# frankenz/Deep-convolutional-neural-network-ResNet-26-and-Attention-network

Measured on AMD Instinct MI355X. Metric: tiles/sec fwd+bwd, 256x256x3 bags, ResNet-26+attn, higher is better.
Workload: dtype bf16; 1 GPU; 8 bags x 256 tiles @256x256x3 per GPU, ResNet-26 (20/40/60/80) + attention-MIL head, fwd+bwd full-bag path (BASELINE.json configs[1]); global_bags=8, tiles_per_bag=256, tile=256, parallelism=bag-parallel dp1, one RCCL all-reduce of the flat 2.56 MB gradient bucket

## Files before the change

### deep-convolutional-neural-network-resnet-26-and-attention-network_amd/csrc/conv_bwd_fused.hip

```cpp
#include "pf_common.cuh"
#include "reduce.cuh"
#include <cstdlib>

struct BwdFusedArgs {
    const __bf16* dz;
    const __bf16* w;
    const __bf16* x;
    const __bf16* addend;
    __bf16* dx;
    float* slab;
    ConvGeom g;
    int ntiles;
    int lds_w_off, lds_x_off, lds_dump_off, lds_a2_off;
    int lds_x2_off;
    int apply_mask;
    float slope;
    unsigned z_bytes, x_bytes;
    unsigned g_bytes;
    int gpx;
    int xpx;
    unsigned long long* stamp;
};

#ifdef MIL_STAMP
// ... 399 lines not shown
                slab[(size_t)(mt * 16 + gq * 4 + e) * SLAB_COLS + nt * 16 + r] = wacc[i][nt][e];
        if (i == bias_i && r == 0) {
#pragma unroll
            for (int e = 0; e < 4; ++e) {
                const int row = mt * 16 + gq * 4 + e;
                const int co = row - CTAP * CZ;
                if (co >= 0 && co < CZ) slab[(size_t)MT * 16 * SLAB_COLS + co] = bacc[e];
            }
        }
    }
}


template <bool ADD, bool MASK>
__global__ __launch_bounds__(512, 4) void conv_bwd_fused16_kernel(BwdFusedArgs a) {
    extern __shared__ __attribute__((aligned(16))) char smem[];
    MIL_POISON(smem);
    constexpr int CZ = 24, NTX = 2, KS = 3, NW = 8;
    constexpr int PIXB = 48, PIXX = 48, CX = 24, HW = 18, ROWB = HW * PIXB;
    constexpr int KSTEPS_STD = 7;
    constexpr int NTHR = 512, MTW = 2, KSTEPS = MIL_K20_STEPS, MT = 12, MW = 2;
    constexpr int NPX = 4;
    constexpr int HALO0 = 16;
    const ConvGeom& g = a.g;
    const int tid = threadIdx.x, lane = tid & 63;
    const int wave = __builtin_amdgcn_readfirstlane(tid >> 6);
    const int r = lane & 15, gq = lane >> 4;
    char* ldsW = smem + a.lds_w_off;
    {
        mil_stage_filter(ldsW, reinterpret_cast<const char*>(a.w) + KSTEPS_STD * NTX * 64 * 16, KSTEPS * NTX * 64 * 16, tid, NTHR);
        if (tid < 2) *reinterpret_cast<u32x2_t*>(smem + tid * a.lds_a2_off + HALO0 + (HW * HW - 1) * PIXB + 40) = u32x2_t{0u, 0u};
    }
    const __amdgpu_buffer_rsrc_t rs_z = mil_rsrc(a.dz, a.z_bytes);
    const __amdgpu_buffer_rsrc_t rs_x = mil_rsrc(a.x, a.x_bytes);
    const __amdgpu_buffer_rsrc_t rs_add = mil_rsrc(a.addend, a.addend ? a.g_bytes : 0);
    const __amdgpu_buffer_rsrc_t rs_dx = mil_rsrc(a.dx, a.g_bytes);
    const int H = g.H, W = g.W, GPX = a.gpx;

    int h_pos[NPX];
    const int h_j8 = (tid & 3) * 8;
    const int h_lds0 = (tid >> 2) * PIXB + h_j8;
#pragma unroll
    for (int i = 0; i < NPX; ++i) {
        const int px = i < 3 ? (tid >> 2) + 128 * i : tid;
        const int hy = px / HW, hx = px - hy * HW;
        h_pos[i] = px < HW * HW ? (hy << 10) | hx : (int)0x80000000u;
    }
    u32x2_t rx[NPX];
    auto fetch_halo = [&](const TileOrigin& o) {
        const int iy0 = o.oy0 - 1, ix0 = o.ox0 - 1;
        const int base = ((o.img0 * H + iy0) * W + ix0) * GPX;
#pragma unroll
        for (int i = 0; i < NPX; ++i) {
            int p = h_pos[i];
            asm volatile("" : "+v"(p));
            const int hy = (p >> 10) & 1023, hx = p & 1023;
            const bool ok = (p >= 0) & ((unsigned)(iy0 + hy) < (unsigned)H) & ((unsigned)(ix0 + hx) < (unsigned)W);
            const int rel = (hy * W + hx) * GPX + (i < 3 ? h_j8 : 32);
            rx[i] = __builtin_amdgcn_raw_buffer_load_b64(rs_z, ok ? (unsigned)(base + rel) : MIL_OOB, 0, 0);
        }
    };

    auto koff = [](int q) { return mil_k20_off(q, ROWB, PIXB); };
    const int bA = (wave * MTW * HW + r) * PIXB + 16 * gq;
    int zb[KSTEPS];
#pragma unroll
    for (int sl = 0; sl < KSTEPS; ++sl) {
        const int o0 = koff(4 * sl);
        const int d1 = koff(4 * sl + 1) - o0 - 16, d2 = koff(4 * sl + 2) - o0 - 32, d3 = koff(4 * sl + 3) - o0 - 48;
        zb[sl] = bA + (gq == 1 ? d1 : gq == 2 ? d2 : gq == 3 ? d3 : 0);
    }
    const int e_ty = wave * MTW + (gq & 1);
    const int c_off = (gq >> 1) * 16;
    const int x_lds = (e_ty * 16 + r) * PIXX + c_off;
    const bool last_ok = (gq >> 1) == 0;
    const int q4 = (lane & 15) >> 2, p4 = lane & 3;
    int zw[MW][2];
    {
        const int kl0 = 8 * gq + q4, kl1 = kl0 + 4;
        const int wpl0 = ((kl0 >> 4) * HW + (kl0 & 15)) * PIXB, wpl1 = ((kl1 >> 4) * HW + (kl1 & 15)) * PIXB;
#pragma unroll
        for (int i = 0; i < MW; ++i) {
            int P = 4 * (wave + NW * i) + p4;
            if (P >= KS * KS * 5) P = 0;
            const int tap = P / 5, c4 = P - tap * 5;
            const int wt = ((tap / KS) * HW + (tap % KS)) * PIXB + c4 * 8;
            zw[i][0] = wpl0 + wt; zw[i][1] = wpl1 + wt;
        }
    }
    const int xb = (8 * gq + q4) * PIXX + p4 * 8;
    f32x4_t wacc[MW][NTX];
#pragma unroll
    for (int i = 0; i < MW; ++i)
#pragma unroll
        for (int nt = 0; nt < NTX; ++nt) wacc[i][nt] = f32x4_t{0.f, 0.f, 0.f, 0.f};

    TileWalker cur, nxt;
    const int bid = mil_xcd_block_id();
    cur.init(g, bid, gridDim.x);
    nxt = cur; nxt.advance();
    if (bid < a.ntiles) fetch_halo(cur.origin(g));
    unsigned goff = MIL_OOB, goff_n = MIL_OOB;
    u32x4_t rxc0, radd0;
    u32x2_t rxc1, radd1;
    auto fetch_x = [&](const TileOrigin& o) {
        const int opix = (o.img0 * H + o.oy0 + e_ty) * W + o.ox0 + r;
        const bool ok = e_ty < H - o.oy0 && r < W - o.ox0;
        const unsigned xoff = ok ? (unsigned)(opix * (CX * 2) + c_off) : MIL_OOB;
        goff_n = ok ? (unsigned)(opix * GPX + c_off) : MIL_OOB;
        rxc0 = __builtin_amdgcn_raw_buffer_load_b128(rs_x, xoff, 0, 0);
        rxc1 = __builtin_amdgcn_raw_buffer_load_b64(rs_x, last_ok ? xoff + 32 : MIL_OOB, 0, 0);
    };
    auto fetch_add = [&]() {
        if constexpr (ADD) {
            radd0 = __builtin_amdgcn_raw_buffer_load_b128(rs_add, goff_n, 0, 0);
            radd1 = __builtin_amdgcn_raw_buffer_load_b64(rs_add, last_ok ? goff_n + 32 : MIL_OOB, 0, 0);
        }
    };
    if (bid < a.ntiles) { fetch_x(cur.origin(g)); fetch_add(); }

    const int buf_step = a.lds_a2_off, xbuf_step = a.lds_x2_off;
    int buf = 0, xbuf = 0;
    MIL_ST_DECL
    for (int tile = bid; tile < a.ntiles; tile += gridDim.x) {
        MIL_ST_BEGIN()
        char* ldsA_t = smem + buf + HALO0;
        char* ldsX_t = smem + a.lds_x_off + xbuf;
        buf = buf_step - buf;
        xbuf = xbuf_step - xbuf;
        {
            int p2 = h_pos[2], p3 = h_pos[3];
            asm volatile("" : "+v"(p2), "+v"(p3));
            *reinterpret_cast<u32x2_t*>(ldsA_t + h_lds0) = rx[0];
            *reinterpret_cast<u32x2_t*>(ldsA_t + h_lds0 + 128 * PIXB) = rx[1];
            *reinterpret_cast<u32x2_t*>(ldsA_t + (p2 >= 0 ? h_lds0 + 256 * PIXB : -16)) = rx[2];
            const int l3 = p3 >= 0 ? tid * PIXB + 32 : -16;
            *reinterpret_cast<u32x2_t*>(ldsA_t + l3) = rx[3];
            *reinterpret_cast<u32x2_t*>(ldsA_t + (p3 >= 0 ? l3 - 40 : -8)) = rx[3];
        }
        *reinterpret_cast<u32x4_t*>(ldsX_t + x_lds) = rxc0;
        *reinterpret_cast<u32x4_t*>(last_ok ? ldsX_t + x_lds + 32 : smem + a.lds_dump_off) = u32x4_t{rxc1[0], rxc1[1], 0u, 0x3f800000u};
        goff = goff_n;
        MIL_ST_MARK(0)
        __syncthreads();
        MIL_ST_MARK(1)
        const bool more = tile + (int)gridDim.x < a.ntiles;
        if (more) { const TileOrigin o_next = nxt.origin(g); fetch_halo(o_next); fetch_x(o_next); }
        cur = nxt; nxt.advance();
        u32x4_t mk0;
        u32x2_t mk1;
        if constexpr (MASK) {
            mk0 = *reinterpret_cast<const u32x4_t*>(ldsX_t + x_lds);
            mk1 = *reinterpret_cast<const u32x2_t*>(last_ok ? ldsX_t + x_lds + 32 : smem + a.lds_dump_off);
        }

        f32x4_t acc[MTW][NTX];
#pragma unroll
        for (int m = 0; m < MTW; ++m)
#pragma unroll
            for (int nt = 0; nt < NTX; ++nt) acc[m][nt] = f32x4_t{0.f, 0.f, 0.f, 0.f};
        {
            Frag8<BF16> wc[NTX], zc[MTW], wn[NTX], zn[MTW];
#pragma unroll
            for (int nt = 0; nt < NTX; ++nt) wc[nt] = lds_frag<BF16>(ldsW + (nt * 64 + lane) * 16);
#pragma unroll
            for (int m = 0; m < MTW; ++m) zc[m] = lds_frag<BF16>(ldsA_t + zb[0] + koff(0) + m * ROWB);
#pragma unroll
            for (int sl = 0; sl < KSTEPS; ++sl) {
                if (sl + 1 < KSTEPS) {
#pragma unroll
                    for (int nt = 0; nt < NTX; ++nt) wn[nt] = lds_frag<BF16>(ldsW + (((sl + 1) * NTX + nt) * 64 + lane) * 16);
#pragma unroll
                    for (int m = 0; m < MTW; ++m) zn[m] = lds_frag<BF16>(ldsA_t + zb[sl + 1] + koff(4 * (sl + 1)) + m * ROWB);
                }
                __builtin_amdgcn_sched_barrier(0);
#pragma unroll
                for (int m = 0; m < MTW; ++m)
#pragma unroll
                    for (int nt = 0; nt < NTX; ++nt) acc[m][nt] = mma8(wc[nt], zc[m], acc[m][nt]);
                __builtin_amdgcn_sched_barrier(0);
#pragma unroll
                for (int nt = 0; nt < NTX; ++nt) wc[nt] = wn[nt];
#pragma unroll
                for (int m = 0; m < MTW; ++m) zc[m] = zn[m];
            }
        }
        MIL_ST_MARK(2)

        {
            float v[8];
#pragma unroll
            for (int i = 0; i < 4; ++i) {
                float lo = acc[0][0][i], hi = acc[1][0][i];
                if (i == 0) mil_swap16<true>(lo, hi); else mil_swap16<false>(lo, hi);
                v[i] = lo;
                v[4 + i] = hi;
            }
            if constexpr (ADD) {
                const bf16x8_t t = __builtin_bit_cast(bf16x8_t, radd0);
#pragma unroll
                for (int i = 0; i < 8; ++i) v[i] += (float)t[i];
            }
            if constexpr (MASK) {
                const bf16x8_t t = __builtin_bit_cast(bf16x8_t, mk0);
#pragma unroll
                for (int i = 0; i < 8; ++i) v[i] *= ((float)t[i] > 0.f ? 1.f : a.slope);
            }
            bf16x8_t ov;
#pragma unroll
            for (int i = 0; i < 8; ++i) ov[i] = (__bf16)v[i];
            __builtin_amdgcn_raw_buffer_store_b128(__builtin_bit_cast(u32x4_t, ov), rs_dx, goff, 0, 0);
        }
        {
            float v[4];
#pragma unroll
            for (int i = 0; i < 4; ++i) {
                float lo = acc[0][1][i], hi = acc[1][1][i];
                if (i == 0) mil_swap16<true>(lo, hi); else mil_swap16<false>(lo, hi);
                v[i] = lo;
            }
            if constexpr (ADD) {
                const bf16x4_t t = __builtin_bit_cast(bf16x4_t, radd1);
#pragma unroll
                for (int i = 0; i < 4; ++i) v[i] += (float)t[i];
            }
            if constexpr (MASK) {
                const bf16x4_t t = __builtin_bit_cast(bf16x4_t, mk1);
#pragma unroll
                for (int i = 0; i < 4; ++i) v[i] *= ((float)t[i] > 0.f ? 1.f : a.slope);
            }
            bf16x4_t ov;
#pragma unroll
            for (int i = 0; i < 4; ++i) ov[i] = (__bf16)v[i];
            const u32x2_t ou = __builtin_bit_cast(u32x2_t, ov);
            const unsigned off = last_ok ? goff + 32 : MIL_OOB;
            if (GPX == 48) __builtin_amdgcn_raw_buffer_store_b128(u32x4_t{ou[0], ou[1], 0u, 0u}, rs_dx, off, 0, 0);
            else __builtin_amdgcn_raw_buffer_store_b64(ou, rs_dx, off, 0, 0);
        }
        MIL_ST_MARK(3)
        if (more) fetch_add();
        MIL_ST_MARK(4)

        {
            bf16x8_t xc[NTX], zc[MW], xn[NTX], zn[MW];
#pragma unroll
            for (int nt = 0; nt < NTX; ++nt) xc[nt] = mil_tr_pair(ldsX_t + xb + nt * 32, ldsX_t + xb + nt * 32 + 4 * PIXX);
#pragma unroll
            for (int i = 0; i < MW; ++i) zc[i] = mil_tr_pair(ldsA_t + zw[i][0], ldsA_t + zw[i][1]);
#pragma unroll
            for (int kk = 0; kk < 8; ++kk) {
                if (kk + 1 < 8) {
#pragma unroll
                    for (int nt = 0; nt < NTX; ++nt)
                        xn[nt] = mil_tr_pair(ldsX_t + xb + (kk + 1) * 32 * PIXX + nt * 32, ldsX_t + xb + (kk + 1) * 32 * PIXX + nt * 32 + 4 * PIXX);
#pragma unroll
                    for (int i = 0; i < MW; ++i)
                        zn[i] = mil_tr_pair(ldsA_t + zw[i][0] + (kk + 1) * 2 * ROWB, ldsA_t + zw[i][1] + (kk + 1) * 2 * ROWB);
                }
                __builtin_amdgcn_sched_barrier(0);
#pragma unroll
                for (int i = 0; i < MW; ++i) {
                    if (i == MW - 1 && wave + NW * i >= MT) continue;
#pragma unroll
                    for (int nt = 0; nt < NTX; ++nt)
                        wacc[i][nt] = __builtin_amdgcn_mfma_f32_16x16x32_bf16(zc[i], xc[nt], wacc[i][nt], 0, 0, 0);
                }
                __builtin_amdgcn_sched_barrier(0);
#pragma unroll
                for (int nt = 0; nt < NTX; ++nt) xc[nt] = xn[nt];
#pragma unroll
                for (int i = 0; i < MW; ++i) zc[i] = zn[i];
            }
        }
        MIL_ST_MARK(5)
#ifdef MIL_STAMP
        ++st_tiles;
#endif
    }
#ifdef MIL_STAMP
    if (a.stamp && lane == 0) {
        unsigned long long* d = a.stamp + ((size_t)blockIdx.x * NW + wave) * 8;
#pragma unroll
        for (int i = 0; i < 6; ++i) d[i] = st_sum[i];
        d[6] = (unsigned long long)st_tiles;
        d[7] = __builtin_amdgcn_s_memrealtime() - st_rt0;
    }
#endif
    constexpr int SLAB_COLS = NTX * 16;
    constexpr size_t SLAB_ELEMS = (size_t)(14 + 1) * 16 * SLAB_COLS;
    float* slab = a.slab + (size_t)blockIdx.x * SLAB_ELEMS;
#pragma unroll
    for (int i = 0; i < MW; ++i) {
        const int mt = wave + NW * i;
        if (mt >= MT) continue;
#pragma unroll
        for (int nt = 0; nt < NTX; ++nt)
#pragma unroll
            for (int e = 0; e < 4; ++e)
                slab[(size_t)(mt * 16 + gq * 4 + e) * SLAB_COLS + nt * 16 + r] = wacc[i][nt][e];
    }
}

#include "conv_bwd_fused16_x3.cuh"


template <typename T, int CZ, int NTX, int KS, int NW = 4>
static int run_bwd_fused(BwdFusedArgs a, float* dw, float* db, void* ws, size_t ws_bytes, int cout, int cin, int accumulate, bool query,
                         size_t* need, hipStream_t stream, bool dense_grads = false) {
    constexpr int ESZ = T::ESZ, EM = ESZ / 2;
    constexpr int PIXB = mil_pix_pitch(CZ, ESZ);
    constexpr int CX = mil_nt_to_cp(NTX);
    constexpr int PIXX = mil_pix_pitch(CX, ESZ);
    constexpr int DUMPA = T::SPLIT ? CZ * 2 + 16 : 16, DUMPX = T::SPLIT ? CX * 2 + 16 : 16;
    constexpr int KSTEPS = (KS * KS * (CZ / 8) + 3) / 4;
    constexpr int RG = KS * KS * (CZ / 8);
    constexpr int MT = (RG + 1) / 2;
    mil_geom_tiles(a.g, 8);
    {
        const int px = (a.g.hh * a.g.hw) << a.g.ti_log2;
        const int need = ((px * PIXB + 15) & ~15) + DUMPA + KSTEPS * NTX * 64 * 8 * ESZ + 256 * PIXX + DUMPX;
        if (need > 160 * 1024 && a.g.tw_log2 == 3 && a.g.ti_log2 == 2 && (a.g.Wo > 8 || a.g.Ho > 8)) mil_geom_set(a.g, 4, 4, 0);
    }
    const int halo_px = (a.g.hh * a.g.hw) << a.g.ti_log2;
    if (halo_px > 400 || a.g.hh >= 1024 || a.g.hw >= 1024) return MIL_ERR_UNSUPPORTED;
    const size_t img_bytes = (size_t)a.g.H * a.g.W * (CZ > CX ? CZ : CX) * ESZ;
    int chunk = mil_imgs_under_2g(img_bytes);
    if (chunk >= 16) chunk &= ~15;
    const int n_total = a.g.n_img;
    if (chunk < n_total) { a.g.n_img = chunk; a.g.n_groups = (chunk + (1 << a.g.ti_log2) - 1) >> a.g.ti_log2; }
    const int a_bytes = ((halo_px * PIXB + 15) & ~15) + DUMPA;
    const int w_bytes = KSTEPS * NTX * 64 * 8 * ESZ;
    const int x_bytes = 256 * PIXX;
    const bool dbuf = 2 * (2 * a_bytes + w_bytes + x_bytes + DUMPX) <= 160 * 1024;
    bool t16 = false;
    if constexpr (CZ == 24 && NTX == 2 && KS == 3 && NW == 8 && !T::SPLIT)
        t16 = dbuf && a.g.tw_log2 == 4 && a.g.th_log2 == 4 && a.g.ti_log2 == 0 && a.g.H < 1024 && a.g.W < 1024 &&
              cout == 20;
    if (dense_grads && !t16) return MIL_ERR_UNSUPPORTED;
    const int lds = (dbuf ? 2 : 1) * a_bytes + w_bytes + (t16 ? 2 : 1) * x_bytes + DUMPX;
    if (lds > 160 * 1024) return MIL_ERR_UNSUPPORTED;
    const int ntiles = a.g.n_groups * a.g.tiles_y * a.g.tiles_x;
    auto kern = a.addend ? (a.apply_mask ? conv_bwd_fused_kernel<T, CZ, NTX, KS, true, true, NW> : conv_bwd_fused_kernel<T, CZ, NTX, KS, true, false, NW>)
                         : (a.apply_mask ? conv_bwd_fused_kernel<T, CZ, NTX, KS, false, true, NW> : conv_bwd_fused_kernel<T, CZ, NTX, KS, false, false, NW>);
    if constexpr (CZ == 24 && NTX == 2 && KS == 3 && NW == 8 && !T::SPLIT) {
        if (t16) kern = a.addend ? (a.apply_mask ? conv_bwd_fused16_kernel<true, true> : conv_bwd_fused16_kernel<true, false>)
                                 : (a.apply_mask ? conv_bwd_fused16_kernel<false, true> : conv_bwd_fused16_kernel<false, false>);
    }
    if (lds > 64 * 1024) {
        if (hipFuncSetAttribute(reinterpret_cast<const void*>(kern), hipFuncAttributeMaxDynamicSharedMemorySize, lds) != hipSuccess)
            return MIL_ERR_LAUNCH;
    }
    int per_cu = 3;
    {
        int o1 = mil_resident_per_cu(conv_bwd_fused_kernel<T, CZ, NTX, KS, true, true, NW>, lds, 3, 64 * NW);
        int o2 = mil_resident_per_cu(conv_bwd_fused_kernel<T, CZ, NTX, KS, false, true, NW>, lds, 3, 64 * NW);
        int o3 = mil_resident_per_cu(conv_bwd_fused_kernel<T, CZ, NTX, KS, true, false, NW>, lds, 3, 64 * NW);
        if constexpr (CZ == 24 && NTX == 2 && KS == 3 && NW == 8 && !T::SPLIT) {
            if (t16) {
                o1 = mil_resident_per_cu(conv_bwd_fused16_kernel<true, true>, lds, 3, 512);
                o2 = mil_resident_per_cu(conv_bwd_fused16_kernel<false, true>, lds, 3, 512);
                o3 = mil_resident_per_cu(conv_bwd_fused16_kernel<true, false>, lds, 3, 512);
            }
        }
        per_cu = o1 < o2 ? o1 : o2; per_cu = per_cu < o3 ? per_cu : o3;
    }
    int grid = mil_num_cus() * per_cu;
    if (grid > ntiles) grid = ntiles;
    const size_t slab_elems = (size_t)(MT + 1) * 16 * NTX * 16;
    size_t bytes = slab_elems * grid * sizeof(float);
#ifdef MIL_STAMP
    const size_t stamp_off = (bytes + 15) & ~(size_t)15;
    bytes = stamp_off + (size_t)grid * NW * 8 * sizeof(unsigned long long);
#endif
    if (query) { *need = bytes; return MIL_OK; }
    if (!ws || ws_bytes < bytes) return MIL_ERR_ARG;
#ifdef MIL_STAMP
    a.stamp = reinterpret_cast<unsigned long long*>(reinterpret_cast<char*>(ws) + stamp_off);
#endif
    const int a_tot = (dbuf ? 2 : 1) * a_bytes;
    a.slab = (float*)ws; a.lds_w_off = a_tot; a.lds_x_off = a_tot + w_bytes; a.lds_dump_off = a_tot + w_bytes + x_bytes * (t16 ? 2 : 1);
    a.lds_a2_off = dbuf ? a_bytes : 0;
    a.lds_x2_off = t16 ? x_bytes : 0;
    if (grid <= 0) return MIL_OK;
    const int n_rows = KS * KS * CZ;
    const BwdFusedArgs a0 = a;
    for (int i0 = 0; i0 < n_total; i0 += chunk) {
        const int n = n_total - i0 < chunk ? n_total - i0 : chunk;
        BwdFusedArgs c = a0;
        c.g.n_img = n;
        c.g.n_groups = (n + (1 << c.g.ti_log2) - 1) >> c.g.ti_log2;
        c.ntiles = c.g.n_groups * c.g.tiles_y * c.g.tiles_x;
        const int gz = dense_grads ? 20 : CZ, gx = dense_grads ? 20 : CX;
        const size_t zo = (size_t)i0 * a.g.H * a.g.W * gz, xo = (size_t)i0 * a.g.H * a.g.W * CX, go = (size_t)i0 * a.g.H * a.g.W * gx;
        c.dz = a0.dz + zo * EM; c.x = a0.x + xo * EM; c.dx = a0.dx + go * EM;
        if (a0.addend) c.addend = a0.addend + go * EM;
        c.z_bytes = (unsigned)((size_t)n * a.g.H * a.g.W * gz * ESZ);
        c.x_bytes = (unsigned)((size_t)n * a.g.H * a.g.W * CX * ESZ);
        c.g_bytes = (unsigned)((size_t)n * a.g.H * a.g.W * gx * ESZ);
        c.gpx = gz * 2;
        int gr = grid < c.ntiles ? grid : c.ntiles;
        hipLaunchKernelGGL(kern, dim3(gr), dim3(64 * NW), lds, stream, c);
        MIL_CHECK_LAUNCH();
        {
            MilReduceJob j{};
            j.slab = (const float*)ws; j.nslab = gr; j.slab_elems = slab_elems; j.slab_cols = NTX * 16; j.n_rows = n_rows;
            j.dw = dw; j.db = db; j.cout = cout; j.cin = cin; j.ks = KS; j.kind = 1; j.cinp = CZ;
            j.bias_off = t16 ? (KS * KS / 2) * CZ * NTX * 16 + (CX - 1) : MT * 16 * NTX * 16; j.bias_stride = t16 ? NTX * 16 : 1;
            if (t16) {
                j.cinp = 20; j.n_rows = KS * KS * 20; j.bias_off = (KS * KS / 2) * 20 * NTX * 16 + (CX - 1);
            }
            j.accumulate = (i0 > 0) ? 1 : accumulate;
            mil_reduce_or_defer(j, stream, chunk >= n_total);
        }
        MIL_CHECK_LAUNCH();
    }
    return MIL_OK;
}

static int run_bwd_fused16_x3(BwdFusedArgs a, float* dw, float* db, void* ws, size_t ws_bytes, int cout, int cin, int accumulate, bool query,
                              size_t* need, hipStream_t stream, bool dense_grads) {
    constexpr int KS = 3, NTX = 2, MT_PITCH = 14;
    if (cout != 20 || cin != 20) return MIL_ERR_UNSUPPORTED;
    mil_geom_tiles(a.g, 8);
    if (a.g.tw_log2 != 4 || a.g.th_log2 != 4 || a.g.ti_log2 != 0 || a.g.H >= 1024 || a.g.W >= 1024) return MIL_ERR_UNSUPPORTED;
    constexpr int A_PLANE = 16 + 18 * 18 * 48, X_PLANE = 256 * 48, W_BYTES = MIL_K20_STEPS * NTX * 64 * 32;
    constexpr int lds = 2 * A_PLANE + W_BYTES + 2 * X_PLANE + 64;
    const int gpx = dense_grads ? 80 : 96, xpx = 96;
    const size_t img_bytes = (size_t)a.g.H * a.g.W * 96;
    int chunk = mil_imgs_under_2g(img_bytes);
    if (chunk >= 16) chunk &= ~15;
    const int n_total = a.g.n_img;
    if (chunk < n_total) { a.g.n_img = chunk; a.g.n_groups = chunk; }
    const int ntiles = a.g.n_groups * a.g.tiles_y * a.g.tiles_x;
    auto pick = [](bool add, bool mask) {
        return add ? (mask ? conv_bwd_fused16x3_kernel<true, true> : conv_bwd_fused16x3_kernel<true, false>)
                   : (mask ? conv_bwd_fused16x3_kernel<false, true> : conv_bwd_fused16x3_kernel<false, false>);
    };
    auto kern = pick(a.addend != nullptr, a.apply_mask != 0);
    static std::atomic<unsigned long long> attr_set{0};
    if (mil_device_needs(attr_set)) {
        for (int v = 0; v < 4; ++v)
            if (hipFuncSetAttribute(reinterpret_cast<const void*>(pick(v & 1, v & 2)), hipFuncAttributeMaxDynamicSharedMemorySize, lds) != hipSuccess)
                return MIL_ERR_LAUNCH;
        mil_device_done(attr_set);
    }
    int per_cu = 3;
    for (int v = 0; v < 4; ++v) {
        const int o = mil_resident_per_cu(pick(v & 1, v & 2), lds, 3, 256);
        per_cu = o < per_cu ? o : per_cu;
    }
    int grid = mil_num_cus() * per_cu;
    if (grid > ntiles) grid = ntiles;
    const size_t slab_elems = (size_t)(MT_PITCH + 1) * 16 * NTX * 16;
    const size_t bytes = slab_elems * grid * sizeof(float);
    if (query) { *need = bytes; return MIL_OK; }
    if (!ws || ws_bytes < bytes) return MIL_ERR_ARG;
    a.slab = (float*)ws;
    a.lds_w_off = 2 * A_PLANE; a.lds_x_off = 2 * A_PLANE + W_BYTES; a.lds_dump_off = 2 * A_PLANE + W_BYTES + 2 * X_PLANE;
    a.lds_a2_off = 0; a.lds_x2_off = 0;
    if (grid <= 0) return MIL_OK;
    const BwdFusedArgs a0 = a;
    for (int i0 = 0; i0 < n_total; i0 += chunk) {
        const int n = n_total - i0 < chunk ? n_total - i0 : chunk;
        BwdFusedArgs c = a0;
        c.g.n_img = n; c.g.n_groups = n;
        c.ntiles = n * c.g.tiles_y * c.g.tiles_x;
        const size_t px0 = (size_t)i0 * a.g.H * a.g.W, npx = (size_t)n * a.g.H * a.g.W;
        c.dz = a0.dz + px0 * gpx / 2; c.x = a0.x + px0 * xpx / 2; c.dx = a0.dx + px0 * gpx / 2;
        if (a0.addend) c.addend = a0.addend + px0 * gpx / 2;
        c.z_bytes = (unsigned)(npx * gpx); c.g_bytes = (unsigned)(npx * gpx); c.x_bytes = (unsigned)(npx * xpx);
        c.gpx = gpx; c.xpx = xpx;
        const int gr = grid < c.ntiles ? grid : c.ntiles;
#ifdef MIL_STAMP
        static MilStampBuf sb;
        c.stamp = sb.get((size_t)gr * 4 * 10);
#endif
        hipLaunchKernelGGL(kern, dim3(gr), dim3(256), lds, stream, c);
        MIL_CHECK_LAUNCH();
#ifdef MIL_STAMP
        static const char* const ph[8] = {"barrier-top", "commit", "barrier-vis", "fetch-issue", "dgrad", "epilogue", "addend-issue", "wgrad"};
        sb.report(a0.addend ? "conv_bwd_fused16x3_kernel<ADD>" : "conv_bwd_fused16x3_kernel", gr, 4, 8, ph, stream);
#endif
        MilReduceJob j{};
        j.slab = (const float*)ws; j.nslab = gr; j.slab_elems = slab_elems; j.slab_cols = NTX * 16;
        j.dw = dw; j.db = db; j.cout = cout; j.cin = cin; j.ks = KS; j.kind = 1;
        j.cinp = 20; j.n_rows = KS * KS * 20; j.bias_off = (KS * KS / 2) * 20 * NTX * 16 + 23; j.bias_stride = NTX * 16;
        j.accumulate = (i0 > 0) ? 1 : accumulate;
        mil_reduce_or_defer(j, stream, chunk >= n_total);
        MIL_CHECK_LAUNCH();
    }
    return MIL_OK;
}

static int bwd_fused_entry(const void* dz, const void* wpack, const void* x, const void* addend, void* dx, float* dw,
                           float* db, void* ws, size_t ws_bytes, int n_img, int H, int W, int cout, int cin, int ks,
                           int pad, int apply_mask, int accumulate, float slope, int dtype, bool query, size_t* need, void* stream) {
    const bool dense_grads = dtype == MIL_DT_BF16_DGRAD || dtype == MIL_DT_F32S_DGRAD;
    if ((dtype != MIL_DT_BF16 && !dense_grads && dtype != MIL_DT_F32S) || ks != 3 || pad != 1) return MIL_ERR_UNSUPPORTED;
    if (n_img <= 0 || H <= 0 || W <= 0) return MIL_ERR_ARG;
    if (slope <= 0.f || slope >= 1.f) return MIL_ERR_UNSUPPORTED;
    BwdFusedArgs a{};
    a.dz = (const __bf16*)dz; a.w = (const __bf16*)wpack; a.x = (const __bf16*)x; a.addend = (const __bf16*)addend;
    a.dx = (__bf16*)dx; a.apply_mask = apply_mask; a.slope = slope;
    a.g.n_img = n_img; a.g.H = H; a.g.W = W; a.g.Ho = H; a.g.Wo = W; a.g.ks = ks; a.g.stride = 1; a.g.pad = pad; a.g.zins = 0;
    const int czp = mil_cpad(cout), cxp = mil_cpad(cin);
    hipStream_t st = reinterpret_cast<hipStream_t>(stream);
    if (dtype == MIL_DT_F32S || dtype == MIL_DT_F32S_DGRAD) {
        if (czp != 24 || cxp != 24) return MIL_ERR_UNSUPPORTED;
        const int rc = run_bwd_fused16_x3(a, dw, db, ws, ws_bytes, cout, cin, accumulate, query, need, st, dense_grads);
        if (rc != MIL_ERR_UNSUPPORTED || dense_grads) return rc;
        return run_bwd_fused<F32S, 24, 2, 3, 8>(a, dw, db, ws, ws_bytes, cout, cin, accumulate, query, need, st);
    }
    if (czp == 24 && cxp == 24) return run_bwd_fused<BF16, 24, 2, 3, 8>(a, dw, db, ws, ws_bytes, cout, cin, accumulate, query, need, st, dense_grads);
    if (dense_grads) return MIL_ERR_UNSUPPORTED;
    if (czp == 40 && cxp == 40) return run_bwd_fused<BF16, 40, 3, 3, 8>(a, dw, db, ws, ws_bytes, cout, cin, accumulate, query, need, st);
    if (czp == 64 && cxp == 64) return run_bwd_fused<BF16, 64, 4, 3, 8>(a, dw, db, ws, ws_bytes, cout, cin, accumulate, query, need, st);
    return MIL_ERR_UNSUPPORTED;
}

extern "C" int mil_conv_bwd_fused_workspace(size_t* bytes, int n_img, int H, int W, int cout, int cin, int ks, int pad,
                                            int dtype) {
    if (!bytes) return MIL_ERR_ARG;
    return bwd_fused_entry(nullptr, nullptr, nullptr, nullptr, nullptr, nullptr, nullptr, nullptr, 0, n_img, H, W, cout, cin,
                           ks, pad, 0, 0, 0.1f, dtype, true, bytes, nullptr);
}

extern "C" int mil_conv_bwd_fused(const void* dz, const void* wpack_dgrad, const void* x, const void* addend, void* dx,
                                  float* dw, float* db, void* workspace, size_t workspace_bytes, int n_img, int H, int W,
                                  int cout, int cin, int ks, int pad, int apply_mask, int accumulate, float slope, int dtype,
                                  void* stream) {
    if (!dz || !wpack_dgrad || !x || !dx || !dw) return MIL_ERR_ARG;
    size_t need = 0;
    return bwd_fused_entry(dz, wpack_dgrad, x, addend, dx, dw, db, workspace, workspace_bytes, n_img, H, W, cout, cin, ks,
                           pad, apply_mask, accumulate, slope, dtype, false, &need, stream);
}
```

Measured before the change: 254,300 tiles/s.

## Add specialized 16x16-tile fused backward conv kernel for 40-channel layers

Adds a dedicated fused backward kernel for 3x3 convs with 40 input and 40 output channels. It uses a 16x16 spatial tile, a double-buffered halo and x tiles in LDS, and register prefetch of the next tile. The kernel computes dx plus the weight and bias gradients in one pass, aiming to cut generic-kernel overhead and improve reuse for the stage-2 layers. It also relaxes the double-buffer condition so single-workgroup-per-CU double buffering is allowed when two workgroups would not fit, trading occupancy for overlap. An env knob can disable the new path.

Result: no change. 255,900 tiles/s, median of 6 (+0.6%).

```diff
diff --git a/deep-convolutional-neural-network-resnet-26-and-attention-network_amd/csrc/conv_bwd_fused.hip b/deep-convolutional-neural-network-resnet-26-and-attention-network_amd/csrc/conv_bwd_fused.hip
--- a/deep-convolutional-neural-network-resnet-26-and-attention-network_amd/csrc/conv_bwd_fused.hip
+++ b/deep-convolutional-neural-network-resnet-26-and-attention-network_amd/csrc/conv_bwd_fused.hip
@@ -725,6 +725,13 @@
 }
 
 #include "conv_bwd_fused16_x3.cuh"
+#include "conv_bwd_fused16c40.cuh"
+
+static bool mil_bwd40_tile16_wanted(int H, int W, int cout, int cin) {
+    if (cout != 40 || cin != 40 || (H & 15) || (W & 15) || H >= 1024 || W >= 1024) return false;
+    const char* e = mil_test_knob("MIL_BWD40_TILE16");
+    return !(e && e[0] == '0');
+}
 
 
 template <typename T, int CZ, int NTX, int KS, int NW = 4>
@@ -744,6 +751,11 @@
         const int need = ((px * PIXB + 15) & ~15) + DUMPA + KSTEPS * NTX * 64 * 8 * ESZ + 256 * PIXX + DUMPX;
         if (need > 160 * 1024 && a.g.tw_log2 == 3 && a.g.ti_log2 == 2 && (a.g.Wo > 8 || a.g.Ho > 8)) mil_geom_set(a.g, 4, 4, 0);
     }
+    bool t40 = false;
+    if constexpr (CZ == 40 && NTX == 3 && KS == 3 && NW == 8 && !T::SPLIT) {
+        t40 = mil_bwd40_tile16_wanted(a.g.H, a.g.W, cout, cin);
+        if (t40) mil_geom_set(a.g, 4, 4, 0);
+    }
     const int halo_px = (a.g.hh * a.g.hw) << a.g.ti_log2;
     if (halo_px > 400 || a.g.hh >= 1024 || a.g.hw >= 1024) return MIL_ERR_UNSUPPORTED;
     const size_t img_bytes = (size_t)a.g.H * a.g.W * (CZ > CX ? CZ : CX) * ESZ;
@@ -754,13 +766,14 @@
     const int a_bytes = ((halo_px * PIXB + 15) & ~15) + DUMPA;
     const int w_bytes = KSTEPS * NTX * 64 * 8 * ESZ;
     const int x_bytes = 256 * PIXX;
-    const bool dbuf = 2 * (2 * a_bytes + w_bytes + x_bytes + DUMPX) <= 160 * 1024;
+    const int lds_1 = a_bytes + w_bytes + x_bytes + DUMPX, lds_2 = lds_1 + a_bytes;
+    const bool dbuf = 2 * lds_2 <= 160 * 1024 || (2 * lds_1 > 160 * 1024 && lds_2 <= 160 * 1024);
     bool t16 = false;
     if constexpr (CZ == 24 && NTX == 2 && KS == 3 && NW == 8 && !T::SPLIT)
         t16 = dbuf && a.g.tw_log2 == 4 && a.g.th_log2 == 4 && a.g.ti_log2 == 0 && a.g.H < 1024 && a.g.W < 1024 &&
               cout == 20;
     if (dense_grads && !t16) return MIL_ERR_UNSUPPORTED;
-    const int lds = (dbuf ? 2 : 1) * a_bytes + w_bytes + (t16 ? 2 : 1) * x_bytes + DUMPX;
+    const int lds = t40 ? MIL_C40_LDS : (dbuf ? 2 : 1) * a_bytes + w_bytes + (t16 ? 2 : 1) * x_bytes + DUMPX;
     if (lds > 160 * 1024) return MIL_ERR_UNSUPPORTED;
     const int ntiles = a.g.n_groups * a.g.tiles_y * a.g.tiles_x;
     auto kern = a.addend ? (a.apply_mask ? conv_bwd_fused_kernel<T, CZ, NTX, KS, true, true, NW> : conv_bwd_fused_kernel<T, CZ, NTX, KS, true, false, NW>)
@@ -768,6 +781,10 @@
     if constexpr (CZ == 24 && NTX == 2 && KS == 3 && NW == 8 && !T::SPLIT) {
         if (t16) kern = a.addend ? (a.apply_mask ? conv_bwd_fused16_kernel<true, true> : conv_bwd_fused16_kernel<true, false>)
                                  : (a.apply_mask ? conv_bwd_fused16_kernel<false, true> : conv_bwd_fused16_kernel<false, false>);
+    }
+    if constexpr (CZ == 40 && NTX == 3 && KS == 3 && NW == 8 && !T::SPLIT) {
+        if (t40) kern = a.addend ? (a.apply_mask ? conv_bwd_fused16c40_kernel<true, true> : conv_bwd_fused16c40_kernel<true, false>)
+                                 : (a.apply_mask ? conv_bwd_fused16c40_kernel<false, true> : conv_bwd_fused16c40_kernel<false, false>);
     }
     if (lds > 64 * 1024) {
         if (hipFuncSetAttribute(reinterpret_cast<const void*>(kern), hipFuncAttributeMaxDynamicSharedMemorySize, lds) != hipSuccess)
@@ -783,6 +800,13 @@
                 o1 = mil_resident_per_cu(conv_bwd_fused16_kernel<true, true>, lds, 3, 512);
                 o2 = mil_resident_per_cu(conv_bwd_fused16_kernel<false, true>, lds, 3, 512);
                 o3 = mil_resident_per_cu(conv_bwd_fused16_kernel<true, false>, lds, 3, 512);
+            }
+        }
+        if constexpr (CZ == 40 && NTX == 3 && KS == 3 && NW == 8 && !T::SPLIT) {
+            if (t40) {
+                o1 = mil_resident_per_cu(conv_bwd_fused16c40_kernel<true, true>, lds, 3, 512);
+                o2 = mil_resident_per_cu(conv_bwd_fused16c40_kernel<false, true>, lds, 3, 512);
+                o3 = mil_resident_per_cu(conv_bwd_fused16c40_kernel<true, false>, lds, 3, 512);
             }
         }
         per_cu = o1 < o2 ? o1 : o2; per_cu = per_cu < o3 ? per_cu : o3;
diff --git a/deep-convolutional-neural-network-resnet-26-and-attention-network_amd/csrc/conv_bwd_fused16c40.cuh b/deep-convolutional-neural-network-resnet-26-and-attention-network_amd/csrc/conv_bwd_fused16c40.cuh
--- /dev/null
+++ b/deep-convolutional-neural-network-resnet-26-and-attention-network_amd/csrc/conv_bwd_fused16c40.cuh
@@ -0,0 +1,263 @@
+#pragma once
+
+constexpr int MIL_C40_PIX = 80;
+constexpr int MIL_C40_A_BYTES = 18 * 18 * MIL_C40_PIX + 16;
+constexpr int MIL_C40_W_BYTES = 12 * 3 * 64 * 16;
+constexpr int MIL_C40_X_BYTES = 256 * MIL_C40_PIX;
+constexpr int MIL_C40_W_OFF = 2 * MIL_C40_A_BYTES;
+constexpr int MIL_C40_X_OFF = MIL_C40_W_OFF + MIL_C40_W_BYTES;
+constexpr int MIL_C40_DUMP_OFF = MIL_C40_X_OFF + 2 * MIL_C40_X_BYTES;
+constexpr int MIL_C40_LDS = MIL_C40_DUMP_OFF + 16;
+static_assert(MIL_C40_LDS <= 160 * 1024, "one workgroup per CU");
+
+__host__ __device__ constexpr int mil_c40_koff(int q) { return q >= 45 ? 0 : (q / 15) * (18 * MIL_C40_PIX) + (q % 15) * 16; }
+
+template <bool ADD, bool MASK>
+__global__ __launch_bounds__(512, 2) void conv_bwd_fused16c40_kernel(BwdFusedArgs a) {
+    extern __shared__ __attribute__((aligned(16))) char smem[];
+    MIL_POISON(smem);
+    constexpr int CZ = 40, NTX = 3, KS = 3, NW = 8, NTHR = 512;
+    constexpr int PIXB = MIL_C40_PIX, PIXX = MIL_C40_PIX, HW = 18, ROWB = HW * PIXB;
+    constexpr int MTW = 2, KSTEPS = 12, CG = 5, RG = KS * KS * CG, MT = (RG + 1) / 2, MW = 3;
+    constexpr int NPX = 4;
+    constexpr int A_DUMP = HW * HW * PIXB;
+    const ConvGeom& g = a.g;
+    const int tid = threadIdx.x, lane = tid & 63;
+    const int wave = __builtin_amdgcn_readfirstlane(tid >> 6);
+    const int r = lane & 15, gq = lane >> 4;
+    char* ldsW = smem + MIL_C40_W_OFF;
+    mil_stage_filter(ldsW, a.w, MIL_C40_W_BYTES, tid, NTHR);
+    if (tid == 0) *reinterpret_cast<u32x4_t*>(smem + MIL_C40_X_OFF + MIL_C40_X_BYTES) = u32x4_t{0u, 0u, 0u, 0u};
+
+    const __amdgpu_buffer_rsrc_t rs_z = mil_rsrc(a.dz, a.z_bytes);
+    const __amdgpu_buffer_rsrc_t rs_x = mil_rsrc(a.x, a.x_bytes);
+    const __amdgpu_buffer_rsrc_t rs_add = mil_rsrc(a.addend, a.addend ? a.x_bytes : 0);
+    const __amdgpu_buffer_rsrc_t rs_dx = mil_rsrc(a.dx, a.x_bytes);
+    const int H = g.H, W = g.W;
+
+    int h_pos[NPX], h_rel[NPX];
+#pragma unroll
+    for (int i = 0; i < NPX; ++i) {
+        const int id = tid + NTHR * i;
+        const int px = id / CG, j = id - px * CG;
+        const int hy = px / HW, hx = px - hy * HW;
+        h_pos[i] = px < HW * HW ? (hy << 10) | hx : (int)0x80000000u;
+        h_rel[i] = (hy * W + hx) * (CZ * 2) + j * 16;
+    }
+    u32x4_t rx[NPX];
+    auto fetch_halo = [&](const TileOrigin& o) {
+        const int iy0 = o.oy0 - 1, ix0 = o.ox0 - 1;
+        const int base = ((o.img0 * H + iy0) * W + ix0) * (CZ * 2);
+#pragma unroll
+        for (int i = 0; i < NPX; ++i) {
+            const int p = h_pos[i];
+            const int hy = (p >> 10) & 1023, hx = p & 1023;
+            const bool ok = (p >= 0) & ((unsigned)(iy0 + hy) < (unsigned)H) & ((unsigned)(ix0 + hx) < (unsigned)W);
+            rx[i] = __builtin_amdgcn_raw_buffer_load_b128(rs_z, ok ? (unsigned)(base + h_rel[i]) : MIL_OOB, 0, 0);
+        }
+    };
+    const int h_lds3 = h_pos[3] >= 0 ? (tid + 3 * NTHR) * 16 : A_DUMP;
+
+    const int bA = (wave * MTW * HW + r) * PIXB + 16 * gq;
+    int zb[KSTEPS];
+#pragma unroll
+    for (int sl = 0; sl < KSTEPS; ++sl) {
+        const int o0 = mil_c40_koff(4 * sl);
+        const int d1 = mil_c40_koff(4 * sl + 1) - o0 - 16, d2 = mil_c40_koff(4 * sl + 2) - o0 - 32, d3 = mil_c40_koff(4 * sl + 3) - o0 - 48;
+        zb[sl] = bA + (gq == 1 ? d1 : gq == 2 ? d2 : gq == 3 ? d3 : 0);
+    }
+    const int e_ty = wave * MTW + (gq & 1);
+    const int c_off = (gq >> 1) * 16;
+    const int x_lds = (e_ty * 16 + r) * PIXX + c_off;
+    const bool last_ok = (gq >> 1) == 0;
+    const int x_lds2 = last_ok ? MIL_C40_X_OFF + x_lds + 64 : MIL_C40_DUMP_OFF;
+    const int q4 = (lane & 15) >> 2, p4 = lane & 3;
+    int zw[MW][2];
+    {
+        const int kl0 = 8 * gq + q4, kl1 = kl0 + 4;
+        const int wpl0 = ((kl0 >> 4) * HW + (kl0 & 15)) * PIXB, wpl1 = ((kl1 >> 4) * HW + (kl1 & 15)) * PIXB;
+#pragma unroll
+        for (int i = 0; i < MW; ++i) {
+            int rg = 2 * (wave + NW * i) + (p4 >> 1);
+            if (rg >= RG) rg = 0;
+            const int tap = rg / CG, cg = rg - tap * CG;
+            const int wt = ((tap / KS) * HW + (tap % KS)) * PIXB + cg * 16 + (p4 & 1) * 8;
+            zw[i][0] = wpl0 + wt; zw[i][1] = wpl1 + wt;
+        }
+    }
+    const int xb = (8 * gq + q4) * PIXX + p4 * 8;
+    const bool has_bias = wave >= 2 && wave <= 4;
+    f32x4_t wacc[MW][NTX];
+    f32x4_t bacc = f32x4_t{0.f, 0.f, 0.f, 0.f};
+#pragma unroll
+    for (int i = 0; i < MW; ++i)
+#pragma unroll
+        for (int nt = 0; nt < NTX; ++nt) wacc[i][nt] = f32x4_t{0.f, 0.f, 0.f, 0.f};
+    bf16x8_t ones;
+#pragma unroll
+    for (int j = 0; j < 8; ++j) ones[j] = (__bf16)1.0f;
+
+    TileWalker cur, nxt;
+    const int bid = mil_xcd_block_id();
+    cur.init(g, bid, gridDim.x);
+    nxt = cur; nxt.advance();
+    unsigned goff = MIL_OOB, goff_n = MIL_OOB;
+    u32x4_t rxc[NTX], radd[NTX];
+    auto fetch_x = [&](const TileOrigin& o) {
+        const int opix = (o.img0 * H + o.oy0 + e_ty) * W + o.ox0 + r;
+        const bool ok = e_ty < H - o.oy0 && r < W - o.ox0;
+        goff_n = ok ? (unsigned)(opix * (CZ * 2) + c_off) : MIL_OOB;
+        rxc[0] = __builtin_amdgcn_raw_buffer_load_b128(rs_x, goff_n, 0, 0);
+        rxc[1] = __builtin_amdgcn_raw_buffer_load_b128(rs_x, goff_n + 32, 0, 0);
+        rxc[2] = __builtin_amdgcn_raw_buffer_load_b128(rs_x, last_ok ? goff_n + 64 : MIL_OOB, 0, 0);
+    };
+    auto fetch_add = [&]() {
+        if constexpr (ADD) {
+            radd[0] = __builtin_amdgcn_raw_buffer_load_b128(rs_add, goff_n, 0, 0);
+            radd[1] = __builtin_amdgcn_raw_buffer_load_b128(rs_add, goff_n + 32, 0, 0);
+            radd[2] = __builtin_amdgcn_raw_buffer_load_b128(rs_add, last_ok ? goff_n + 64 : MIL_OOB, 0, 0);
+        }
+    };
+    if (bid < a.ntiles) { const TileOrigin o0 = cur.origin(g); fetch_halo(o0); fetch_x(o0); fetch_add(); }
+
+    int buf = 0, xbuf = 0;
+    for (int tile = bid; tile < a.ntiles; tile += gridDim.x) {
+        char* ldsA_t = smem + buf;
+        char* ldsX_t = smem + MIL_C40_X_OFF + xbuf;
+        char* x2_t = smem + x_lds2 + (last_ok ? xbuf : 0);
+        buf = MIL_C40_A_BYTES - buf;
+        xbuf = MIL_C40_X_BYTES - xbuf;
+        *reinterpret_cast<u32x4_t*>(ldsA_t + tid * 16) = rx[0];
+        *reinterpret_cast<u32x4_t*>(ldsA_t + (tid + NTHR) * 16) = rx[1];
+        *reinterpret_cast<u32x4_t*>(ldsA_t + (tid + 2 * NTHR) * 16) = rx[2];
+        *reinterpret_cast<u32x4_t*>(ldsA_t + h_lds3) = rx[3];
+        *reinterpret_cast<u32x4_t*>(ldsX_t + x_lds) = rxc[0];
+        *reinterpret_cast<u32x4_t*>(ldsX_t + x_lds + 32) = rxc[1];
+        *reinterpret_cast<u32x4_t*>(x2_t) = rxc[2];
+        goff = goff_n;
+        __syncthreads();
+        const bool more = tile + (int)gridDim.x < a.ntiles;
+        if (more) { const TileOrigin o_next = nxt.origin(g); fetch_halo(o_next); fetch_x(o_next); }
+        cur = nxt; nxt.advance();
+        u32x4_t mk[NTX];
+        if constexpr (MASK) {
+            mk[0] = *reinterpret_cast<const u32x4_t*>(ldsX_t + x_lds);
+            mk[1] = *reinterpret_cast<const u32x4_t*>(ldsX_t + x_lds + 32);
+            mk[2] = *reinterpret_cast<const u32x4_t*>(x2_t);
+        }
+
+        f32x4_t acc[MTW][NTX];
+#pragma unroll
+        for (int m = 0; m < MTW; ++m)
+#pragma unroll
+            for (int nt = 0; nt < NTX; ++nt) acc[m][nt] = f32x4_t{0.f, 0.f, 0.f, 0.f};
+        {
+            Frag8<BF16> wc[NTX], zc[MTW], wn[NTX], zn[MTW];
+#pragma unroll
+            for (int nt = 0; nt < NTX; ++nt) wc[nt] = lds_frag<BF16>(ldsW + (nt * 64 + lane) * 16);
+#pragma unroll
+            for (int m = 0; m < MTW; ++m) zc[m] = lds_frag<BF16>(ldsA_t + zb[0] + mil_c40_koff(0) + m * ROWB);
+#pragma unroll
+            for (int sl = 0; sl < KSTEPS; ++sl) {
+                if (sl + 1 < KSTEPS) {
+#pragma unroll
+                    for (int nt = 0; nt < NTX; ++nt) wn[nt] = lds_frag<BF16>(ldsW + (((sl + 1) * NTX + nt) * 64 + lane) * 16);
+#pragma unroll
+                    for (int m = 0; m < MTW; ++m) zn[m] = lds_frag<BF16>(ldsA_t + zb[sl + 1 < KSTEPS ? sl + 1 : sl] + mil_c40_koff(4 * (sl + 1)) + m * ROWB);
+                }
+                __builtin_amdgcn_sched_barrier(0);
+#pragma unroll
+                for (int m = 0; m < MTW; ++m)
+#pragma unroll
+                    for (int nt = 0; nt < NTX; ++nt) acc[m][nt] = mma8(wc[nt], zc[m], acc[m][nt]);
+                __builtin_amdgcn_sched_barrier(0);
+#pragma unroll
+                for (int nt = 0; nt < NTX; ++nt) wc[nt] = wn[nt];
+#pragma unroll
+                for (int m = 0; m < MTW; ++m) zc[m] = zn[m];
+            }
+        }
+
+#pragma unroll
+        for (int nt = 0; nt < NTX; ++nt) {
+            float v[8];
+#pragma unroll
+            for (int i = 0; i < 4; ++i) {
+                float lo = acc[0][nt][i], hi = acc[1][nt][i];
+                if (i == 0) mil_swap16<true>(lo, hi); else mil_swap16<false>(lo, hi);
+                v[i] = lo;
+                v[4 + i] = hi;
+            }
+            if constexpr (ADD) {
+                const bf16x8_t t = __builtin_bit_cast(bf16x8_t, radd[nt]);
+#pragma unroll
+                for (int i = 0; i < 8; ++i) v[i] += (float)t[i];
+            }
+            if constexpr (MASK) {
+                const bf16x8_t t = __builtin_bit_cast(bf16x8_t, mk[nt]);
+#pragma unroll
+                for (int i = 0; i < 8; ++i) v[i] *= ((float)t[i] > 0.f ? 1.f : a.slope);
+            }
+            bf16x8_t ov;
+#pragma unroll
+            for (int i = 0; i < 8; ++i) ov[i] = (__bf16)v[i];
+            const unsigned off = (nt == NTX - 1 && !last_ok) ? MIL_OOB : goff + nt * 32;
+            __builtin_amdgcn_raw_buffer_store_b128(__builtin_bit_cast(u32x4_t, ov), rs_dx, off, 0, 0);
+        }
+        if (more) fetch_add();
+
+        {
+            bf16x8_t xc[NTX], zc[MW], xn[NTX], zn[MW];
+#pragma unroll
+            for (int nt = 0; nt < NTX; ++nt) xc[nt] = mil_tr_pair(ldsX_t + xb + nt * 32, ldsX_t + xb + nt * 32 + 4 * PIXX);
+#pragma unroll
+            for (int i = 0; i < MW; ++i) zc[i] = mil_tr_pair(ldsA_t + zw[i][0], ldsA_t + zw[i][1]);
+#pragma unroll
+            for (int kk = 0; kk < 8; ++kk) {
+                if (kk + 1 < 8) {
+#pragma unroll
+                    for (int nt = 0; nt < NTX; ++nt)
+                        xn[nt] = mil_tr_pair(ldsX_t + xb + (kk + 1) * 32 * PIXX + nt * 32, ldsX_t + xb + (kk + 1) * 32 * PIXX + nt * 32 + 4 * PIXX);
+#pragma unroll
+                    for (int i = 0; i < MW; ++i)
+                        zn[i] = mil_tr_pair(ldsA_t + zw[i][0] + (kk + 1) * 2 * ROWB, ldsA_t + zw[i][1] + (kk + 1) * 2 * ROWB);
+                }
+                __builtin_amdgcn_sched_barrier(0);
+#pragma unroll
+                for (int i = 0; i < MW; ++i) {
+                    if (i == MW - 1 && wave + NW * i >= MT) continue;
+#pragma unroll
+                    for (int nt = 0; nt < NTX; ++nt)
+                        wacc[i][nt] = __builtin_amdgcn_mfma_f32_16x16x32_bf16(zc[i], xc[nt], wacc[i][nt], 0, 0, 0);
+                    if (i == 1 && has_bias) bacc = __builtin_amdgcn_mfma_f32_16x16x32_bf16(zc[i], ones, bacc, 0, 0, 0);
+                }
+                __builtin_amdgcn_sched_barrier(0);
+#pragma unroll
+                for (int nt = 0; nt < NTX; ++nt) xc[nt] = xn[nt];
+#pragma unroll
+                for (int i = 0; i < MW; ++i) zc[i] = zn[i];
+            }
+        }
+    }
+
+    constexpr int SLAB_COLS = NTX * 16;
+    constexpr size_t SLAB_ELEMS = (size_t)(MT + 1) * 16 * SLAB_COLS;
+    float* slab = a.slab + (size_t)blockIdx.x * SLAB_ELEMS;
+#pragma unroll
+    for (int i = 0; i < MW; ++i) {
+        const int mt = wave + NW * i;
+        if (mt >= MT) continue;
+#pragma unroll
+        for (int nt = 0; nt < NTX; ++nt)
+#pragma unroll
+            for (int e = 0; e < 4; ++e)
+                slab[(size_t)(mt * 16 + gq * 4 + e) * SLAB_COLS + nt * 16 + r] = wacc[i][nt][e];
+        if (i == 1 && has_bias && r == 0) {
+#pragma unroll
+            for (int e = 0; e < 4; ++e) {
+                const int co = mt * 16 + gq * 4 + e - (KS * KS / 2) * CZ;
+                if (co >= 0 && co < CZ) slab[(size_t)MT * 16 * SLAB_COLS + co] = bacc[e];
+            }
+        }
+    }
+}
```
